# miuda-ai/lele

Hardware: AMD Instinct MI355X
Metric: STFT+mel GB/s (SenseVoice front-end: PCM -> log-mel -> LFR, algorithmic bytes); SenseVoiceSmall-shaped RTF in `sensevoice` (higher is better)
Workload: dtype f32

## Files before the change

lele_amd/csrc/fe_core.h:

```cpp
#pragma once
#include <stdint.h>

#if defined(__HIPCC__)
#define FE_HD __host__ __device__ __forceinline__
#else
#define FE_HD inline
#endif

namespace fe {

constexpr int kNfft = 512;
constexpr int kFrame = 400;
constexpr int kHop = 160;
constexpr int kBins = 257;
constexpr int kLanes = 16;
constexpr int kRegs = 32;
constexpr int kQ = 25;

FE_HD constexpr int rev4(int x) { return ((x & 1) << 3) | ((x & 2) << 1) | ((x & 4) >> 1) | ((x & 8) >> 3); }
FE_HD constexpr int rev5(int x) {
    return ((x & 1) << 4) | ((x & 2) << 2) | (x & 4) | ((x & 8) >> 2) | ((x & 16) >> 4);
}
FE_HD constexpr int tw_off(int s) { return (1 << (s - 1)) - 1; }

FE_HD float fmul(float a, float b) { return a * b; }
FE_HD float fadd(float a, float b) { return a + b; }
FE_HD float fsub(float a, float b) { return a - b; }
FE_HD float ffma(float a, float b, float c) { return __builtin_fmaf(a, b, c); }

#if defined(__HIPCC__) && defined(__HIP_DEVICE_COMPILE__)
typedef float cf __attribute__((ext_vector_type(2)));
FE_HD cf cmk(float re, float im) { return (cf){re, im}; }
FE_HD cf cadd(cf a, cf b) { return a + b; }
FE_HD cf csub(cf a, cf b) { return a - b; }
FE_HD cf cmulv(cf a, cf b) { return a * b; }
FE_HD cf cfmav(cf a, cf b, cf c) { return __builtin_elementwise_fma(a, b, c); }
FE_HD cf cswap(cf a) { return a.yx; }
FE_HD cf cxx(cf a) { return a.xx; }
#else
struct cf {
    float x, y;
};
FE_HD cf cmk(float re, float im) { return cf{re, im}; }
FE_HD cf cadd(cf a, cf b) { return cf{a.x + b.x, a.y + b.y}; }
FE_HD cf csub(cf a, cf b) { return cf{a.x - b.x, a.y - b.y}; }
FE_HD cf cmulv(cf a, cf b) { return cf{a.x * b.x, a.y * b.y}; }
FE_HD cf cfmav(cf a, cf b, cf c) { return cf{__builtin_fmaf(a.x, b.x, c.x), __builtin_fmaf(a.y, b.y, c.y)}; }
FE_HD cf cswap(cf a) { return cf{a.y, a.x}; }
FE_HD cf cxx(cf a) { return cf{a.x, a.x}; }
#endif

struct Tw {
    cf w, wn;
};
FE_HD Tw make_tw(float wr, float wi) { return Tw{cmk(wr, wi), cmk(-wi, wi)}; }

FE_HD cf tw_mul_fma(const Tw& t, cf o) { return cfmav(cxx(t.w), o, cmulv(t.wn, cswap(o))); }

FE_HD void bfly_fma(const Tw& tw, cf& e, cf& o) {
    cf t = tw_mul_fma(tw, o);
    cf n = csub(e, t);
    e = cadd(e, t);
    o = n;
}
FE_HD void bfly_scalar(float wr, float wi, cf& e, cf& o) {
    float tr = fsub(fmul(wr, o.x), fmul(wi, o.y));
    float ti = fadd(fmul(wr, o.y), fmul(wi, o.x));
    cf t = cmk(tr, ti);
    cf n = csub(e, t);
    e = cadd(e, t);
    o = n;
}
FE_HD void bfly_fma(float wr, float wi, float& er, float& ei, float& o_r, float& oi) {
    cf e = cmk(er, ei), o = cmk(o_r, oi);
    bfly_fma(make_tw(wr, wi), e, o);
    er = e.x;
    ei = e.y;
    o_r = o.x;
    oi = o.y;
}
FE_HD void bfly_scalar(float wr, float wi, float& er, float& ei, float& o_r, float& oi) {
    cf e = cmk(er, ei), o = cmk(o_r, oi);
    bfly_scalar(wr, wi, e, o);
    er = e.x;
    ei = e.y;
    o_r = o.x;
    oi = o.y;
}

template <typename TW>
FE_HD void phase_a(cf* a, const TW& tw_re, const TW& tw_im) {
#pragma unroll
    for (int r = 0; r < kRegs; r += 2) bfly_scalar(tw_re[tw_off(1)], tw_im[tw_off(1)], a[r], a[r + 1]);
#pragma unroll
    for (int b = 0; b < kRegs; b += 4) {
#pragma unroll
        for (int k = 0; k < 2; ++k) bfly_scalar(tw_re[tw_off(2) + k], tw_im[tw_off(2) + k], a[b + k], a[b + 2 + k]);
    }
#pragma unroll
    for (int s = 3; s <= 5; ++s) {
        const int half = 1 << (s - 1);
#pragma unroll
        for (int b = 0; b < kRegs; b += 2 * half) {
#pragma unroll
            for (int k = 0; k < half; ++k)
                bfly_fma(make_tw(tw_re[tw_off(s) + k], tw_im[tw_off(s) + k]), a[b + k], a[b + half + k]);
        }
    }
}

template <typename TW>
FE_HD void phase_a_fast(const float* x, cf* a, const TW& tw_re, const TW& tw_im) {
    float s1[kRegs];
#pragma unroll
    for (int r = 0; r < kRegs; r += 2) {
        if (rev5(r + 1) >= kQ) {
            s1[r] = x[r];
            s1[r + 1] = x[r];
        } else {
            s1[r] = fadd(x[r], x[r + 1]);
            s1[r + 1] = fsub(x[r], x[r + 1]);
        }
    }
    {
        const float wr = tw_re[tw_off(2) + 1], wi = tw_im[tw_off(2) + 1];
#pragma unroll
        for (int b = 0; b < kRegs; b += 4) {
            a[b] = cmk(fadd(s1[b], s1[b + 2]), 0.0f);
            a[b + 2] = cmk(fsub(s1[b], s1[b + 2]), 0.0f);
            const float tr = fmul(wr, s1[b + 3]);
            const float ti = fmul(wi, s1[b + 3]);
            a[b + 1] = cmk(fadd(s1[b + 1], tr), ti);
            a[b + 3] = cmk(fsub(s1[b + 1], tr), -ti);
        }
    }
#pragma unroll
    for (int b = 0; b < kRegs; b += 8) {
#pragma unroll
        for (int k = 0; k < 4; ++k) {
            const float wr = tw_re[tw_off(3) + k], wi = tw_im[tw_off(3) + k];
            if ((k & 1) == 0) {
                const float e = a[b + k].x, o = a[b + 4 + k].x;
                const float tr = fmul(wr, o);
                const float ti = fmul(wi, o);
                a[b + k] = cmk(fadd(e, tr), ti);
                a[b + 4 + k] = cmk(fsub(e, tr), -ti);
            } else {
                bfly_fma(make_tw(wr, wi), a[b + k], a[b + 4 + k]);
            }
        }
    }
#pragma unroll
    for (int s = 4; s <= 5; ++s) {
        const int half = 1 << (s - 1);
#pragma unroll
        for (int b = 0; b < kRegs; b += 2 * half) {
#pragma unroll
            for (int k = 0; k < half; ++k)
                bfly_fma(make_tw(tw_re[tw_off(s) + k], tw_im[tw_off(s) + k]), a[b + k], a[b + half + k]);
        }
    }
}

template <typename TWF>
FE_HD void phase_b(cf* b, int c, int rho, const TWF& twf, float* re256) {
#pragma unroll
    for (int s = 6; s <= 8; ++s) {
        const int hv = 1 << (s - 6);
#pragma unroll
        for (int k = 0; k < hv; ++k) {
            const cf w = twf(tw_off(s) + k * 32 + rho * 16 + c);
            const Tw tw = make_tw(w.x, w.y);
#pragma unroll
            for (int base = 0; base < 16; base += 2 * hv) bfly_fma(tw, b[base + k], b[base + hv + k]);
        }
    }
#pragma unroll
    for (int k = 0; k < 8; ++k) {
        const cf w = twf(tw_off(9) + k * 32 + rho * 16 + c);
        const cf t = tw_mul_fma(make_tw(w.x, w.y), b[8 + k]);
        if (k == 0) *re256 = fsub(b[0].x, t.x);
        b[k] = cadd(b[k], t);
    }
}

FE_HD float power(float re, float im) { return fadd(fmul(re, re), fmul(im, im)); }
FE_HD float power(cf z) {
    cf sq = cmulv(z, z);
    return fadd(sq.x, sq.y);
}

constexpr int kXchgPitch = 17;
FE_HD constexpr int xchg_slot(int v, int c) { return v * kXchgPitch + c; }

}
```

lele_amd/csrc/frontend.hip:

```cpp
#include <type_traits>
#include "common.h"
#include "fe_core.h"

#include <math.h>

#include <algorithm>

using namespace lele;

namespace {

constexpr int kMaxMelRounds = 8;

struct FeDev {
    const float* tw_re;
    const float* tw_im;
    const float2* tw;
    const float* window;
    const float* melw;
    const int* mel_start;
    const int* mel_step_off;
    int mel_rounds;
    int mel_steps;
    int n_mels;
    int lfr_m, lfr_n;
};

struct GridBlock {
    __device__ __forceinline__ unsigned x() const { return blockIdx.x; }
    __device__ __forceinline__ unsigned y() const { return blockIdx.y; }
};
struct SegBlock {
    unsigned bx;
    __device__ __forceinline__ unsigned x() const { return bx; }
    __device__ __forceinline__ unsigned y() const { return 0u; }
};

struct FeSeg {
    int64_t start, len;
    int64_t num_frames, t_lfr;
    int64_t row0;
    int64_t block0;
};

constexpr int kSumRows = 66;
constexpr int kSumPitch = 164;

__global__ __launch_bounds__(64) void fe_frame_sum_kernel(const float* __restrict__ pcm, int64_t utt_stride,
                                                          int64_t pcm_len, int64_t num_frames,
                                                          float* __restrict__ mean_out, int aligned16) {
    __shared__ __attribute__((aligned(16))) float tile[kSumRows * kSumPitch];
    const int lane = threadIdx.x;
    const int64_t f0 = (int64_t)blockIdx.x * 64;
    const float* base = pcm + (int64_t)blockIdx.y * utt_stride;
    const int64_t s0 = f0 * fe::kHop;
    constexpr int kVecPerRow = fe::kHop / 4;
    constexpr int kVecs = kSumRows * kVecPerRow;
    constexpr int kIters = (kVecs + 63) / 64;
    constexpr int kBatch = 14;
    static_assert(kIters % kBatch == 0, "batching");
    for (int b0 = 0; b0 < kIters; b0 += kBatch) {
        float4 st[kBatch];
#pragma unroll
        for (int u = 0; u < kBatch; ++u) {
            const int idx = (b0 + u) * 64 + lane;
            int64_t s = s0 + 4 * (int64_t)idx;
            if (s + 3 >= pcm_len) s = aligned16 ? ((pcm_len - 4) & ~int64_t(3)) : (pcm_len - 4);
            if (s < 0) s = 0;
            const float* src = base + s;
            if (aligned16) {
                st[u] = *reinterpret_cast<const float4*>(src);
            } else {
                st[u] = make_float4(src[0], src[1], src[2], src[3]);
            }
        }
#pragma unroll
        for (int u = 0; u < kBatch; ++u) {
            const int idx = (b0 + u) * 64 + lane;
            if (idx < kVecs) {
                float4 xv = st[u];
                xv.x *= 32768.0f;
                xv.y *= 32768.0f;
                xv.z *= 32768.0f;
                xv.w *= 32768.0f;
                const int row = idx / kVecPerRow, c = idx - row * kVecPerRow;
                *reinterpret_cast<float4*>(&tile[row * kSumPitch + 4 * c]) = xv;
            }
        }
    }
    __syncthreads();
    float sum = 0.0f;
#pragma unroll
    for (int seg = 0; seg < 3; ++seg) {
        const float* rowp = &tile[(lane + seg) * kSumPitch];
        const int nvec = seg < 2 ? kVecPerRow : (fe::kFrame - 2 * fe::kHop) / 4;
#pragma unroll 10
        for (int k = 0; k < nvec; ++k) {
            const float4 r = *reinterpret_cast<const float4*>(rowp + 4 * k);
            sum = sum + r.x;
            sum = sum + r.y;
            sum = sum + r.z;
            sum = sum + r.w;
        }
    }
    const int64_t f = f0 + lane;
    if (f < num_frames) mean_out[(int64_t)blockIdx.y * num_frames + f] = sum / (float)fe::kFrame;
}

constexpr int kFrameXchgFloats = 2 * 16 * fe::kXchgPitch;
constexpr int kWaveLdsFloats = 4 * kFrameXchgFloats;
constexpr int kPStride = 272;

struct TwLds {
    const float2* t;
    __device__ __forceinline__ float2 at(int i) const { return t[i]; }
};

template <int MODE>
__device__ __forceinline__ float lane_rot_prev(float v, int p) {
    if (MODE == 1) {
        return __builtin_bit_cast(float,
                                  __builtin_amdgcn_update_dpp(0, __builtin_bit_cast(int, v), 0x121, 0xf, 0xf, true));
    } else {
        return __shfl(v, (p + 15) & 15, 16);
    }
}

constexpr int kStdMelLen[5] = {3, 4, 6, 10, 17};
constexpr int kStdMelOff[6] = {0, 3, 7, 13, 23, 40};

template <int MODE, bool STDMEL, bool FUSED, int PASSES, bool LOWREG, class Blk>
__device__ __forceinline__ void fe_main_body(const float* __restrict__ pcm, int64_t utt_stride,
                                             int64_t num_frames, int64_t t_lfr,
                                             const float* __restrict__ means, const FeDev& tb,
                                             float* __restrict__ out, float* __restrict__ logmel_out,
                                             int aligned16, float* s_melw, Blk bl) {
    constexpr int FR = 16 * PASSES;
    constexpr int kRows = FR + 2;
    constexpr int kXFloats = FUSED ? (kRows * kSumPitch > 4 * kWaveLdsFloats ? kRows * kSumPitch : 4 * kWaveLdsFloats)
                                   : 4 * kWaveLdsFloats;
    __shared__ float2 s_tw[LOWREG ? 480 : 512];
    __shared__ __attribute__((aligned(16))) float s_x[kXFloats];
    __shared__ float s_mean[64];
    __shared__ int s_mstart[16 * (STDMEL ? 5 : kMaxMelRounds)];
    __shared__ int s_moff[kMaxMelRounds + 1];
    constexpr int kTwBase = LOWREG ? 31 : 0;

    for (int i = threadIdx.x; i < 511 - kTwBase; i += 256) s_tw[i] = tb.tw[i + kTwBase];
    if (!STDMEL)
        for (int i = threadIdx.x; i < tb.mel_steps * 16; i += 256) s_melw[i] = tb.melw[i];
    if (threadIdx.x < tb.mel_rounds * 16) s_mstart[threadIdx.x] = tb.mel_start[threadIdx.x];
    if (threadIdx.x <= tb.mel_rounds) s_moff[threadIdx.x] = tb.mel_step_off[threadIdx.x];
    const int lane = threadIdx.x & 63, wave = threadIdx.x >> 6;
    const int g = lane >> 4, p = lane & 15;
    if (FUSED) {
        const float* ubase = pcm + (int64_t)bl.y() * utt_stride;
        const int64_t s0 = (int64_t)bl.x() * FR * fe::kHop;
        constexpr int kVecPerRow = fe::kHop / 4;
        constexpr int kVecs = kRows * kVecPerRow;
        constexpr int kIters = (kVecs + 255) / 256;
        float4 st[kIters];
#pragma unroll
        for (int u = 0; u < kIters; ++u) {
            const int idx = u * 256 + (int)threadIdx.x;
            int64_t sidx = s0 + 4 * (int64_t)idx;
            if (sidx + 3 >= utt_stride) sidx = aligned16 ? ((utt_stride - 4) & ~int64_t(3)) : (utt_stride - 4);
            if (sidx < 0) sidx = 0;
            const float* src = ubase + sidx;
            if (aligned16)
                st[u] = *reinterpret_cast<const float4*>(src);
            else
                st[u] = make_float4(src[0], src[1], src[2], src[3]);
        }
#pragma unroll
        for (int u = 0; u < kIters; ++u) {
            const int idx = u * 256 + (int)threadIdx.x;
            if (idx < kVecs) {
                float4 xv = st[u];
                xv.x *= 32768.0f;
                xv.y *= 32768.0f;
                xv.z *= 32768.0f;
                xv.w *= 32768.0f;
                const int row = idx / kVecPerRow, c = idx - row * kVecPerRow;
                *reinterpret_cast<float4*>(&s_x[row * kSumPitch + 4 * c]) = xv;
            }
        }
        __syncthreads();
    }
    const int h = fe::rev4(p);
    float* xw = s_x + wave * kWaveLdsFloats;
    float* xf = xw + g * kFrameXchgFloats;
    const float* base = pcm + (int64_t)bl.y() * utt_stride;
    const float* mean_u = means + (int64_t)bl.y() * num_frames;
    const int d_out = tb.n_mels * tb.lfr_m;
    float* out_u = out ? out + (int64_t)bl.y() * t_lfr * d_out : nullptr;
    float* lm_u = logmel_out ? logmel_out + (int64_t)bl.y() * num_frames * tb.n_mels : nullptr;

    float win[fe::kQ];
    if (!LOWREG) {
#pragma unroll
        for (int q = 0; q < fe::kQ; ++q) win[q] = tb.window[p + 16 * q];
    }

    float xr[fe::kQ];
    float mean_next = 0.0f;
    auto issue_loads = [&](int pass) {
        const int64_t f = (int64_t)bl.x() * FR + wave * (4 * PASSES) + pass * 4 + g;
        const int64_t fc = f < num_frames ? f : 0;
        const float* src = base + fc * fe::kHop + p;
        if (!FUSED) mean_next = mean_u[fc];
#pragma unroll
        for (int q = 0; q < fe::kQ; ++q) xr[q] = src[16 * q];
    };
    issue_loads(0);
    if (FUSED) {
        constexpr int kVecPerRow = fe::kHop / 4;
        if (wave == 0 && lane < FR) {
            float sum = 0.0f;
#pragma unroll
            for (int seg = 0; seg < 3; ++seg) {
                const float* rowp = &s_x[(lane + seg) * kSumPitch];
                const int nvec = seg < 2 ? kVecPerRow : (fe::kFrame - 2 * fe::kHop) / 4;
#pragma unroll 10
                for (int k = 0; k < nvec; ++k) {
                    const float4 r = *reinterpret_cast<const float4*>(rowp + 4 * k);
                    sum = sum + r.x;
                    sum = sum + r.y;
                    sum = sum + r.z;
                    sum = sum + r.w;
                }
            }
            s_mean[lane] = sum / (float)fe::kFrame;
        }
    }
    __syncthreads();

    auto run_pass = [&](int pass, auto load_next_c) {
        constexpr bool load_next = decltype(load_next_c)::value;
        const int64_t f = (int64_t)bl.x() * FR + wave * (4 * PASSES) + pass * 4 + g;
        const bool valid = f < num_frames;
        const float mean = FUSED ? s_mean[wave * (4 * PASSES) + pass * 4 + g] : mean_next;
        if (LOWREG) {
            int off = 0;
            asm volatile("" : "+v"(off));
#pragma unroll
            for (int q = 0; q < fe::kQ; ++q) win[q] = tb.window[p + 16 * q + off];
        }

        float v[fe::kQ];
        const float neg_mean = -mean;
#pragma unroll
        for (int q = 0; q < fe::kQ; ++q) v[q] = __builtin_fmaf(xr[q], 32768.0f, neg_mean);
        if (load_next) issue_loads(pass + 1);
        float xin[fe::kRegs];
#pragma unroll
        for (int r = 0; r < fe::kRegs; ++r) xin[r] = 0.0f;
        float k97;
        asm("v_mov_b32 %0, 0x3f7851ec" : "=v"(k97));
#pragma unroll
        for (int q = 0; q < fe::kQ; ++q) {
            const float send = (p == 15 && q > 0) ? v[q > 0 ? q - 1 : 0] : v[q];
            const float prev = lane_rot_prev<MODE>(send, p);
            float y = fe::fsub(v[q], fe::fmul(k97, prev));
            if (q == 0) y = (p == 0) ? v[0] : y;
            xin[fe::rev5(q)] = fe::fmul(y, win[q]);
        }

        fe::cf a[fe::kRegs];
        fe::phase_a_fast(xin, a, tb.tw_re, tb.tw_im);

        float pw[2][8];
        float p256 = 0.0f;
#pragma unroll
        for (int rho = 0; rho < 2; ++rho) {
            __builtin_amdgcn_wave_barrier();
#pragma unroll
            for (int cc = 0; cc < 16; ++cc) {
                const int slot = fe::xchg_slot(h, cc);
                *reinterpret_cast<float2*>(xf + 2 * slot) = make_float2(a[rho * 16 + cc].x, a[rho * 16 + cc].y);
            }
            __builtin_amdgcn_wave_barrier();
            fe::cf bq[16];
#pragma unroll
            for (int vv = 0; vv < 16; ++vv) {
                const float2 t = *reinterpret_cast<const float2*>(xf + 2 * fe::xchg_slot(vv, p));
                bq[vv] = fe::cmk(t.x, t.y);
            }
            __builtin_amdgcn_wave_barrier();
            float re256 = 0.0f;
            fe::phase_b(bq, p, rho, [&](int i) { const float2 w = s_tw[i - kTwBase]; return fe::cmk(w.x, w.y); }, &re256);
            if (rho == 0) p256 = re256;
#pragma unroll
            for (int vv = 0; vv < 8; ++vv) {
                fe::cf z = bq[vv];
                if (vv == 0 && rho == 0) z = fe::cmk(z.x, (p == 0) ? 0.0f : z.y);
                pw[rho][vv] = fe::power(z);
            }
        }
        float* prow = xw + g * kPStride;
        __builtin_amdgcn_wave_barrier();
#pragma unroll
        for (int rho = 0; rho < 2; ++rho)
#pragma unroll
            for (int vv = 0; vv < 8; ++vv) prow[(2 * vv + rho) * 16 + p] = pw[rho][vv];
        if (p == 0) prow[256] = fe::power(p256, 0.0f);
        __builtin_amdgcn_wave_barrier();

        const int fi = (int)f, nfr = (int)num_frames, tl = (int)t_lfr;
        const int pad = (tb.lfr_m - 1) / 2;
        const int fp = fi + pad;
        const int b_first = fp % tb.lfr_n, i_first = fp / tb.lfr_n;

        float vals[STDMEL ? 5 : kMaxMelRounds];
#pragma unroll
        for (int rd = 0; rd < (STDMEL ? 5 : kMaxMelRounds); ++rd) {
            vals[rd] = 0.0f;
            if (!STDMEL && rd >= tb.mel_rounds) continue;
            const int m = rd * 16 + p;
            const int start = s_mstart[m];
            const float* pp = prow + start;
            float acc = 0.0f;
            if (STDMEL) {
                const float* wp = tb.melw + kStdMelOff[rd < 5 ? rd : 0] * 16 + p;
                float w[17];
#pragma unroll
                for (int t = 0; t < 17; ++t)
                    if (t < kStdMelLen[rd < 5 ? rd : 0]) w[t] = wp[t * 16];
#pragma unroll
                for (int t = 0; t < 17; ++t)
                    if (t < kStdMelLen[rd < 5 ? rd : 0]) acc = fe::fadd(acc, fe::fmul(w[t], pp[t]));
            } else {
                const int t0 = s_moff[rd], t1 = s_moff[rd + 1];
                const float* wp = s_melw + t0 * 16 + p;
                const int lim = 256 - start;
#pragma unroll 4
                for (int t = 0; t < t1 - t0; ++t) {
                    const float pv = pp[t < lim ? t : lim];
                    acc = fe::fadd(acc, fe::fmul(wp[t * 16], pv));
                }
            }
            {
                const float l2 = __builtin_amdgcn_logf(fmaxf(acc, 1e-5f));
                const float hi = __builtin_bit_cast(float, 0x3f317217u), lo = __builtin_bit_cast(float, 0x3377d1cfu);
                const float r = fe::fmul(l2, hi);
                vals[rd] = fe::fadd(r, fe::ffma(l2, lo, fe::ffma(l2, hi, -r)));
            }
        }
        if (valid) {
            constexpr int kR = STDMEL ? 5 : kMaxMelRounds;
            auto put = [&](float* dst) {
#pragma unroll
                for (int rd = 0; rd < kR; ++rd)
                    if (rd * 16 + p < tb.n_mels) __builtin_nontemporal_store(vals[rd], &dst[rd * 16]);
            };
            if (lm_u) put(lm_u + (int64_t)fi * tb.n_mels + p);
            if (out_u) {
                int i = i_first;
                for (int b = b_first; b < tb.lfr_m && i >= 0; b += tb.lfr_n, --i)
                    if (i < tl) put(out_u + i * d_out + b * tb.n_mels + p);
                if (fi == 0) {
                    for (int i2 = 0; i2 * tb.lfr_n - pad < 0 && i2 < tl; ++i2)
                        for (int b = 0; b < tb.lfr_m && i2 * tb.lfr_n + b - pad < 0; ++b)
                            put(out_u + i2 * d_out + b * tb.n_mels + p);
                }
                if (fi == nfr - 1) {
                    for (int i2 = tl - 1; i2 >= 0 && i2 * tb.lfr_n + (tb.lfr_m - 1) - pad > fi; --i2)
                        for (int b = tb.lfr_m - 1; b >= 0 && i2 * tb.lfr_n + b - pad > fi; --b)
                            put(out_u + i2 * d_out + b * tb.n_mels + p);
                }
            }
        }
        __builtin_amdgcn_wave_barrier();
    };
#pragma unroll 1
    for (int pass = 0; pass + 1 < PASSES; ++pass) run_pass(pass, std::true_type{});
    run_pass(PASSES - 1, std::false_type{});
}

template <int MODE, bool STDMEL, bool FUSED>
__global__ __launch_bounds__(256) void fe_main_kernel(const float* __restrict__ pcm, int64_t utt_stride, int64_t num_frames, int64_t t_lfr,
                                                      const float* __restrict__ means, FeDev tb, float* __restrict__ out,
                                                      float* __restrict__ logmel_out, int aligned16) {
    extern __shared__ float s_melw[];
    fe_main_body<MODE, STDMEL, FUSED, 4, false>(pcm, utt_stride, num_frames, t_lfr, means, tb, out, logmel_out, aligned16, s_melw,
                                                GridBlock{});
}

template <int MODE, bool STDMEL>
__global__ __launch_bounds__(256) void fe_seg_main_kernel(const float* __restrict__ pcm, const FeSeg* __restrict__ segs,
                                                          const int* __restrict__ blk_seg, FeDev tb, float* __restrict__ out) {
    extern __shared__ float s_melw[];
    const FeSeg s = segs[blk_seg[blockIdx.x]];
    const float* base = pcm + s.start;
    const int aligned16 = (((uintptr_t)base & 15) == 0) && (s.len % 4 == 0);
    fe_main_body<MODE, STDMEL, true, 4, false>(base, s.len, s.num_frames, s.t_lfr, nullptr, tb, out + s.row0 * (tb.n_mels * tb.lfr_m),
                                               nullptr, aligned16, s_melw, SegBlock{(unsigned)(blockIdx.x - s.block0)});
}
__global__ void fe_generic_mean_kernel(const float* __restrict__ pcm, int64_t rows, int64_t num_frames, int64_t pcm_len, int frame_len, int hop,
                                       float* __restrict__ mean) {
    const int64_t f = (int64_t)blockIdx.x * blockDim.x + threadIdx.x;
    if (f >= rows) return;
    const float* src = pcm + (f / num_frames) * pcm_len + (f % num_frames) * hop;
    float sum = 0.0f;
    int j = 0;
    if ((((uintptr_t)src) & 15) == 0) {
        for (; j + 16 <= frame_len; j += 16) {
            float4 v[4];
#pragma unroll
            for (int u = 0; u < 4; ++u) v[u] = *reinterpret_cast<const float4*>(src + j + 4 * u);
#pragma unroll
            for (int u = 0; u < 4; ++u) {
                sum = sum + v[u].x * 32768.0f;
                sum = sum + v[u].y * 32768.0f;
                sum = sum + v[u].z * 32768.0f;
                sum = sum + v[u].w * 32768.0f;
            }
        }
    }
    for (; j < frame_len; ++j) sum = sum + src[j] * 32768.0f;
    mean[f] = sum / (float)frame_len;
}
__global__ void fe_generic_frame_kernel(const float* __restrict__ pcm, const float* __restrict__ mean,
                                        const float* __restrict__ window, int64_t rows, int64_t num_frames, int64_t pcm_len, int frame_len, int hop,
                                        int n_fft, float* __restrict__ frames) {
    const int64_t total = rows * n_fft;
    for (int64_t i = (int64_t)blockIdx.x * blockDim.x + threadIdx.x; i < total; i += (int64_t)gridDim.x * blockDim.x) {
        const int64_t f = i / n_fft;
        const int j = (int)(i - f * n_fft);
        float v = 0.0f;
        if (j < frame_len) {
            const float* src = pcm + (f / num_frames) * pcm_len + (f % num_frames) * hop;
            const float m = mean[f];
            const float cur = fe::fsub(fe::fmul(src[j], 32768.0f), m);
            float y = cur;
            if (j >= 1) y = fe::fsub(cur, fe::fmul(0.97f, fe::fsub(fe::fmul(src[j - 1], 32768.0f), m)));
            v = fe::fmul(y, window[j]);
        }
        frames[i] = v;
    }
}
__global__ void fe_generic_mel_kernel(const float* __restrict__ power, int64_t num_frames, int n_bins, int n_mels,
                                      const int* __restrict__ mstart, const int* __restrict__ moff,
                                      const float* __restrict__ mw, float* __restrict__ logmel) {
    const int64_t total = num_frames * n_mels;
    for (int64_t i = (int64_t)blockIdx.x * blockDim.x + threadIdx.x; i < total; i += (int64_t)gridDim.x * blockDim.x) {
        const int64_t f = i / n_mels;
        const int m = (int)(i - f * n_mels);
        const float* p = power + f * n_bins + mstart[m];
        float acc = 0.0f;
        for (int t = moff[m]; t < moff[m + 1]; ++t) acc = fe::fadd(acc, fe::fmul(mw[t], p[t - moff[m]]));
        logmel[i] = __logf(fmaxf(acc, 1e-5f));
    }
}
#define FE_PAD(i) ((i) + ((i) >> 5))
__global__ __launch_bounds__(256) void fe_generic_fused_kernel(const float* __restrict__ pcm, int64_t pcm_len, int64_t num_frames, int frame_len,
                                                               int hop, int n, int log2n, int fpb, const float* __restrict__ window,
                                                               const float* __restrict__ tw_re_g, const float* __restrict__ tw_im_g, int n_mels,
                                                               const int* __restrict__ mstart, const int* __restrict__ moff,
                                                               const float* __restrict__ mw, const float* __restrict__ means,
                                                               float* __restrict__ logmel) {
    extern __shared__ float gfl[];
    const int nb = n / 2 + 1, span = (fpb - 1) * hop + frame_len;
    float* re = gfl;
    float* im = re + FE_PAD(fpb * n) + 1;
    float* pw = im + FE_PAD(fpb * n) + 1;
    float* sp = pw + fpb * nb;
    float* smean = sp + span;
    const int tid = threadIdx.x;
    const int64_t f0 = (int64_t)blockIdx.x * fpb;
    const int nfr = (int)(num_frames - f0 < fpb ? num_frames - f0 : fpb);
    const float* src = pcm + (int64_t)blockIdx.y * pcm_len + f0 * hop;
    const int have = (nfr - 1) * hop + frame_len;
    for (int i = tid; i < span; i += 256) sp[i] = i < have ? src[i] : 0.0f;
    __syncthreads();
    if (means) {
        if (tid < nfr) smean[tid] = means[(int64_t)blockIdx.y * num_frames + f0 + tid];
    } else if (tid < nfr) {
        const float* fr = sp + tid * hop;
        float sum = 0.0f;
        int j = 0;
        for (; j + 16 <= frame_len; j += 16) {
            float v[16];
#pragma unroll
            for (int u = 0; u < 16; ++u) v[u] = fr[j + u];
#pragma unroll
            for (int u = 0; u < 16; ++u) sum = sum + v[u] * 32768.0f;
        }
        for (; j < frame_len; ++j) sum = sum + fr[j] * 32768.0f;
        smean[tid] = sum / (float)frame_len;
    }
    __syncthreads();
    for (int i = tid; i < fpb * n; i += 256) {
        const int f = i >> log2n, j = i & (n - 1);
        float v = 0.0f;
        if (j < frame_len && f < nfr) {
            const float* fr = sp + f * hop;
            const float m = smean[f];
            const float cur = fe::fsub(fe::fmul(fr[j], 32768.0f), m);
            float y = cur;
            if (j >= 1) y = fe::fsub(cur, fe::fmul(0.97f, fe::fsub(fe::fmul(fr[j - 1], 32768.0f), m)));
            v = fe::fmul(y, window[j]);
        }
        const int r = (int)(__brev((unsigned)j) >> (32 - log2n));
        re[FE_PAD(f * n + r)] = v;
        im[FE_PAD(f * n + r)] = 0.0f;
    }
    __syncthreads();
    for (int s0 = 0; s0 < log2n;) {
        const int R = log2n - s0 >= 3 ? 3 : log2n - s0, h = 1 << s0, gsz = 1 << R, groups = n >> R;
        for (int idx = tid; idx < fpb * groups; idx += 256) {
            const int f = idx / groups, g = idx - f * groups;
            const int lo = g & (h - 1), base = f * n + ((g >> s0) << (s0 + R)) + lo;
            float xr[8], xi[8];
#pragma unroll
            for (int j = 0; j < 8; ++j)
                if (j < gsz) xr[j] = re[FE_PAD(base + j * h)], xi[j] = im[FE_PAD(base + j * h)];
#pragma unroll
            for (int r = 0; r < 3; ++r) {
                if (r >= R) break;
                const int half = h << r, off = half - 1;
#pragma unroll
                for (int j = 0; j < 8; ++j) {
                    if (j >= gsz || (j >> r) & 1) continue;
                    const int k = lo + (j & ((1 << r) - 1)) * h;
                    const float wr = tw_re_g[off + k], wi = tw_im_g[off + k];
                    if (half >= 4)
                        fe::bfly_fma(wr, wi, xr[j], xi[j], xr[j + (1 << r)], xi[j + (1 << r)]);
                    else
                        fe::bfly_scalar(wr, wi, xr[j], xi[j], xr[j + (1 << r)], xi[j + (1 << r)]);
                }
            }
#pragma unroll
            for (int j = 0; j < 8; ++j)
                if (j < gsz) re[FE_PAD(base + j * h)] = xr[j], im[FE_PAD(base + j * h)] = xi[j];
        }
        s0 += R;
        __syncthreads();
    }
    for (int i = tid; i < fpb * nb; i += 256) {
        const int f = i / nb, k = i - f * nb;
        const float r = re[FE_PAD(f * n + k)];
        const float q = (k == 0 || k == nb - 1) ? 0.0f : im[FE_PAD(f * n + k)];
        pw[i] = fe::power(r, q);
    }
    __syncthreads();
    for (int i = tid; i < nfr * n_mels; i += 256) {
        const int f = i / n_mels, m = i - f * n_mels;
        const float* pp = pw + f * nb + mstart[m];
        const float* wp = mw + moff[m];
        const int cnt = moff[m + 1] - moff[m];
        float acc = 0.0f;
        int t = 0;
        for (; t + 8 <= cnt; t += 8) {
            float w8[8], p8[8];
#pragma unroll
            for (int u = 0; u < 8; ++u) w8[u] = wp[t + u], p8[u] = pp[t + u];
#pragma unroll
            for (int u = 0; u < 8; ++u) acc = fe::fadd(acc, fe::fmul(w8[u], p8[u]));
        }
        for (; t < cnt; ++t) acc = fe::fadd(acc, fe::fmul(wp[t], pp[t]));
        logmel[((int64_t)blockIdx.y * num_frames + f0 + f) * n_mels + m] = __logf(fmaxf(acc, 1e-5f));
    }
}
__global__ void fe_generic_lfr_kernel(const float* __restrict__ x, int64_t t, int64_t d, int64_t m, int64_t n,
                                      int64_t t_lfr, float* __restrict__ out) {
    const int64_t d_out = d * m, total = t_lfr * d_out, pad = (m - 1) / 2;
    x += (int64_t)blockIdx.y * t * d;
    out += (int64_t)blockIdx.y * total;
    for (int64_t idx = (int64_t)blockIdx.x * blockDim.x + threadIdx.x; idx < total; idx += (int64_t)gridDim.x * blockDim.x) {
        const int64_t i = idx / d_out, rem = idx - i * d_out, block = rem / d, k = rem - block * d;
        int64_t raw = i * n + block - pad;
        raw = raw < 0 ? 0 : (raw > t - 1 ? t - 1 : raw);
        out[idx] = x[raw * d + k];
    }
}

}

struct LeleFrontend {
    LeleCtx* ctx = nullptr;
    LeleFeatureConfig cfg{};
    int64_t frame_len = 0, hop_len = 0, n_fft = 0;
    bool fast = false;
    bool std_mel = false;
    int dpp_mode = 0;
    bool fused = true;
    const float* g_window = nullptr;
    const int* g_mstart = nullptr;
    const int* g_moff = nullptr;
    const float* g_mw = nullptr;
    FeDev dev{};
    std::vector<void*> allocs;
    DevTables seg_tables;
    bool profiling = false;
    std::vector<hipEvent_t> events;
    size_t events_used = 0;
};

namespace {

static const float PI_F = 3.14159265358979323846264338327950288f;

void host_hann(int64_t size, std::vector<float>& w) {
    w.resize(size);
    if (size == 1) w[0] = 1.0f;
    for (int64_t n = 0; size > 1 && n < size; ++n) w[n] = 0.5f * (1.0f - cosf(2.0f * PI_F * (float)n / (float)(size - 1)));
}

void host_twiddles(int64_t n, std::vector<float>& re, std::vector<float>& im) {
    re.clear();
    im.clear();
    for (int64_t size = 2; size <= n; size *= 2) {
        int64_t half = size / 2, step = n / size;
        for (int64_t k = 0; k < half; ++k) {
            float angle = -2.0f * PI_F * (float)(k * step) / (float)n;
            re.push_back(cosf(angle));
            im.push_back(sinf(angle));
        }
    }
}

float hz_to_mel(float hz) { return 2595.0f * log10f(1.0f + hz / 700.0f); }
float mel_to_hz(float mel) { return 700.0f * (powf(10.0f, mel / 2595.0f) - 1.0f); }

void host_dense_mel(float sr, int64_t n_fft, int64_t n_mels, float f_min, float f_max, float* bank) {
    const int64_t n_freqs = n_fft / 2 + 1;
    const float mel_min = hz_to_mel(f_min), mel_max = hz_to_mel(f_max);
    const float mel_step = (mel_max - mel_min) / (float)(n_mels + 1);
    std::vector<float> hz(n_mels + 2), ff(n_freqs);
    for (int64_t i = 0; i < n_mels + 2; ++i) hz[i] = mel_to_hz(mel_min + (float)i * mel_step);
    for (int64_t i = 0; i < n_freqs; ++i) ff[i] = (float)i * sr / (float)n_fft;
    for (int64_t i = 0; i < n_mels; ++i) {
        const float fl = hz[i], fc = hz[i + 1], fr = hz[i + 2];
        for (int64_t j = 0; j < n_freqs; ++j) {
            const float f = ff[j];
            float val = 0.0f;
            if (f > fl && f < fc)
                val = (f - fl) / (fc - fl);
            else if (f >= fc && f < fr)
                val = (fr - f) / (fr - fc);
            bank[i * n_freqs + j] = val;
        }
    }
}

void host_sparse_mel(float sr, int64_t n_fft, int64_t n_mels, float f_min, std::vector<int>& start,
                     std::vector<std::vector<float>>& w) {
    const int64_t n_freqs = n_fft / 2 + 1;
    std::vector<float> bank((size_t)n_mels * n_freqs);
    host_dense_mel(sr, n_fft, n_mels, f_min, sr / 2.0f, bank.data());
    start.assign(n_mels, 0);
    w.assign(n_mels, {});
    for (int64_t i = 0; i < n_mels; ++i) {
        const float* row = bank.data() + i * n_freqs;
        int64_t s = 0;
        while (s < n_freqs && row[s] == 0.0f) ++s;
        int64_t e = n_freqs;
        while (e > s && row[e - 1] == 0.0f) --e;
        if (s < e) {
            start[i] = (int)s;
            w[i].assign(row + s, row + e);
        }
    }
}

template <typename T>
int upload(LeleFrontend* fe, const std::vector<T>& v, const T** out) {
    void* d = nullptr;
    size_t bytes = std::max<size_t>(v.size() * sizeof(T), 16);
    LELE_HIP_CHECK(hipMalloc(&d, bytes));
    fe->allocs.push_back(d);
    if (!v.empty()) LELE_HIP_CHECK(hipMemcpy(d, v.data(), v.size() * sizeof(T), hipMemcpyHostToDevice));
    *out = (const T*)d;
    return 0;
}

}

extern "C" {

int lele_hip_hann_window(int64_t size, float* out) {
    LELE_REQUIRE(size >= 0 && (out || size == 0), "hann_window: bad argument");
    std::vector<float> w;
    host_hann(size, w);
    if (size) memcpy(out, w.data(), (size_t)size * 4);
    return 0;
}
float lele_hip_hz_to_mel_htk(float hz) { return hz_to_mel(hz); }
float lele_hip_mel_to_hz_htk(float mel) { return mel_to_hz(mel); }
int lele_hip_mel_filterbank(float sample_rate, int64_t n_fft, int64_t n_mels, float f_min, int32_t has_f_max, float f_max, float* out) {
    LELE_REQUIRE(n_fft >= 0 && n_mels >= 0 && (out || n_mels == 0), "mel_filterbank: bad argument");
    if (n_mels) host_dense_mel(sample_rate, n_fft, n_mels, f_min, has_f_max ? f_max : sample_rate / 2.0f, out);
// ... 439 lines not shown
```

Baseline: 1758.

## Transpose FFT exchange layout and pre-gather per-lane twiddles for vectorized LDS loads

The shared-memory exchange buffer is transposed so each lane reads its 16 complex inputs contiguously as float4 loads instead of strided float2 loads. Twiddles for phase B are regathered per (rho, lane) into a padded per-lane table, letting each lane fetch its 15 twiddles with vector loads and split those loads around a sched_barrier to overlap them with butterflies. A waves_per_eu hint is also added to the main kernels to steer register allocation and occupancy. The padded layouts use slightly more LDS, and the occupancy hint may raise register pressure or cause spills.

Measured after the change: 1776 (median of 6 runs). 1.01x the previous value.

```diff
diff --git a/lele_amd/csrc/fe_core.h b/lele_amd/csrc/fe_core.h
--- a/lele_amd/csrc/fe_core.h
+++ b/lele_amd/csrc/fe_core.h
@@ -193,4 +193,46 @@
 constexpr int kXchgPitch = 17;
 FE_HD constexpr int xchg_slot(int v, int c) { return v * kXchgPitch + c; }
 
-}
+constexpr int kXchgPitchT = 18;
+constexpr int kXchgFrameFloats = 2 * 16 * kXchgPitchT;
+FE_HD constexpr int xchg_slot_t(int v, int c) { return c * kXchgPitchT + v; }
+
+constexpr int kTwLanePitch = 18;
+constexpr int kTwLaneN = 16;
+FE_HD constexpr int tw_lane_pos(int s, int k) { return (1 << (s - 6)) - 1 + k; }
+FE_HD constexpr int tw_lane_slot(int rho, int c, int i) { return (rho * 16 + c) * kTwLanePitch + i; }
+FE_HD constexpr int tw_lane_src(int rho, int c, int i) {
+    return i == 0 ? tw_off(6) + rho * 16 + c
+         : i < 3  ? tw_off(7) + (i - 1) * 32 + rho * 16 + c
+         : i < 7  ? tw_off(8) + (i - 3) * 32 + rho * 16 + c
+         : i < 15 ? tw_off(9) + (i - 7) * 32 + rho * 16 + c
+                  : 0;
+}
+
+FE_HD void phase_b_lane_stage(cf* b, const cf* tw, int s) {
+    const int hv = 1 << (s - 6);
+#pragma unroll
+    for (int k = 0; k < hv; ++k) {
+        const cf w = tw[tw_lane_pos(s, k)];
+        const Tw t = make_tw(w.x, w.y);
+#pragma unroll
+        for (int base = 0; base < 16; base += 2 * hv) bfly_fma(t, b[base + k], b[base + hv + k]);
+    }
+}
+FE_HD void phase_b_lane_9(cf* b, const cf* tw, float* re256) {
+#pragma unroll
+    for (int k = 0; k < 8; ++k) {
+        const cf w = tw[tw_lane_pos(9, k)];
+        const cf t = tw_mul_fma(make_tw(w.x, w.y), b[8 + k]);
+        if (k == 0) *re256 = fsub(b[0].x, t.x);
+        b[k] = cadd(b[k], t);
+    }
+}
+FE_HD void phase_b_lane(cf* b, const cf* tw, float* re256) {
+    phase_b_lane_stage(b, tw, 6);
+    phase_b_lane_stage(b, tw, 7);
+    phase_b_lane_stage(b, tw, 8);
+    phase_b_lane_9(b, tw, re256);
+}
+
+}
diff --git a/lele_amd/csrc/frontend.hip b/lele_amd/csrc/frontend.hip
--- a/lele_amd/csrc/frontend.hip
+++ b/lele_amd/csrc/frontend.hip
@@ -107,14 +107,9 @@
     if (f < num_frames) mean_out[(int64_t)blockIdx.y * num_frames + f] = sum / (float)fe::kFrame;
 }
 
-constexpr int kFrameXchgFloats = 2 * 16 * fe::kXchgPitch;
+constexpr int kFrameXchgFloats = fe::kXchgFrameFloats;
 constexpr int kWaveLdsFloats = 4 * kFrameXchgFloats;
 constexpr int kPStride = 272;
-
-struct TwLds {
-    const float2* t;
-    __device__ __forceinline__ float2 at(int i) const { return t[i]; }
-};
 
 template <int MODE>
 __device__ __forceinline__ float lane_rot_prev(float v, int p) {
@@ -139,14 +134,17 @@
     constexpr int kRows = FR + 2;
     constexpr int kXFloats = FUSED ? (kRows * kSumPitch > 4 * kWaveLdsFloats ? kRows * kSumPitch : 4 * kWaveLdsFloats)
                                    : 4 * kWaveLdsFloats;
-    __shared__ float2 s_tw[LOWREG ? 480 : 512];
+    constexpr int kTwLaneSlots = 2 * 16 * fe::kTwLanePitch;
+    __shared__ __attribute__((aligned(16))) float2 s_twl[kTwLaneSlots];
     __shared__ __attribute__((aligned(16))) float s_x[kXFloats];
     __shared__ float s_mean[64];
     __shared__ int s_mstart[16 * (STDMEL ? 5 : kMaxMelRounds)];
     __shared__ int s_moff[kMaxMelRounds + 1];
-    constexpr int kTwBase = LOWREG ? 31 : 0;
-
-    for (int i = threadIdx.x; i < 511 - kTwBase; i += 256) s_tw[i] = tb.tw[i + kTwBase];
+
+    for (int i = threadIdx.x; i < kTwLaneSlots; i += 256) {
+        const int row = i / fe::kTwLanePitch, k = i - row * fe::kTwLanePitch;
+        s_twl[i] = tb.tw[k < fe::kTwLaneN ? fe::tw_lane_src(row >> 4, row & 15, k) : 0];
+    }
     if (!STDMEL)
         for (int i = threadIdx.x; i < tb.mel_steps * 16; i += 256) s_melw[i] = tb.melw[i];
     if (threadIdx.x < tb.mel_rounds * 16) s_mstart[threadIdx.x] = tb.mel_start[threadIdx.x];
@@ -276,19 +274,34 @@
             __builtin_amdgcn_wave_barrier();
 #pragma unroll
             for (int cc = 0; cc < 16; ++cc) {
-                const int slot = fe::xchg_slot(h, cc);
+                const int slot = fe::xchg_slot_t(h, cc);
                 *reinterpret_cast<float2*>(xf + 2 * slot) = make_float2(a[rho * 16 + cc].x, a[rho * 16 + cc].y);
             }
             __builtin_amdgcn_wave_barrier();
-            fe::cf bq[16];
-#pragma unroll
-            for (int vv = 0; vv < 16; ++vv) {
-                const float2 t = *reinterpret_cast<const float2*>(xf + 2 * fe::xchg_slot(vv, p));
-                bq[vv] = fe::cmk(t.x, t.y);
+            fe::cf bq[16], tw[fe::kTwLaneN];
+            const float4* trow = reinterpret_cast<const float4*>(s_twl + fe::tw_lane_slot(rho, p, 0));
+            const float4* xrow = reinterpret_cast<const float4*>(xf + 2 * fe::xchg_slot_t(0, p));
+            auto get_tw = [&](int i) {
+                const float4 w = trow[i];
+                tw[2 * i] = fe::cmk(w.x, w.y);
+                tw[2 * i + 1] = fe::cmk(w.z, w.w);
+            };
+#pragma unroll
+            for (int i = 0; i < 8; ++i) {
+                const float4 t = xrow[i];
+                bq[2 * i] = fe::cmk(t.x, t.y);
+                bq[2 * i + 1] = fe::cmk(t.z, t.w);
+                if (i < 4) get_tw(i);
             }
             __builtin_amdgcn_wave_barrier();
             float re256 = 0.0f;
-            fe::phase_b(bq, p, rho, [&](int i) { const float2 w = s_tw[i - kTwBase]; return fe::cmk(w.x, w.y); }, &re256);
+            fe::phase_b_lane_stage(bq, tw, 6);
+            fe::phase_b_lane_stage(bq, tw, 7);
+            __builtin_amdgcn_sched_barrier(0);
+#pragma unroll
+            for (int i = 4; i < 8; ++i) get_tw(i);
+            fe::phase_b_lane_stage(bq, tw, 8);
+            fe::phase_b_lane_9(bq, tw, &re256);
             if (rho == 0) p256 = re256;
 #pragma unroll
             for (int vv = 0; vv < 8; ++vv) {
@@ -378,7 +391,7 @@
 }
 
 template <int MODE, bool STDMEL, bool FUSED>
-__global__ __launch_bounds__(256) void fe_main_kernel(const float* __restrict__ pcm, int64_t utt_stride, int64_t num_frames, int64_t t_lfr,
+__global__ __launch_bounds__(256) __attribute__((amdgpu_waves_per_eu(STDMEL ? 3 : 1))) void fe_main_kernel(const float* __restrict__ pcm, int64_t utt_stride, int64_t num_frames, int64_t t_lfr,
                                                       const float* __restrict__ means, FeDev tb, float* __restrict__ out,
                                                       float* __restrict__ logmel_out, int aligned16) {
     extern __shared__ float s_melw[];
@@ -387,7 +400,7 @@
 }
 
 template <int MODE, bool STDMEL>
-__global__ __launch_bounds__(256) void fe_seg_main_kernel(const float* __restrict__ pcm, const FeSeg* __restrict__ segs,
+__global__ __launch_bounds__(256) __attribute__((amdgpu_waves_per_eu(STDMEL ? 3 : 1))) void fe_seg_main_kernel(const float* __restrict__ pcm, const FeSeg* __restrict__ segs,
                                                           const int* __restrict__ blk_seg, FeDev tb, float* __restrict__ out) {
     extern __shared__ float s_melw[];
     const FeSeg s = segs[blk_seg[blockIdx.x]];
```
